# cvg/pixel-perfect-sfm

Hardware: AMD Instinct MI355X
Metric: featuremetric residuals+Jacobians evaluated/sec (1M obs) (higher is better)
Workload: dtype f32 horizontal / f64 vertical+normalisation on f16 patches; 1 GPU; BASELINE.json configs[2]: synthetic 200 cams / 200000 points / 1000000 obs featuremetric BA residual+Jacobian evaluation, 128-ch fp16 16x16 patches, SIMPLE_RADIAL, fused six-scalar Jacobian reduction; n_obs=1000000, channels=128, patch=16, obs_per_gpu=1000000, partition=none

## Files before the change

### pixel-perfect-sfm_amd/csrc/pxr_ba_gram.hip

```cpp
#include <hip/hip_runtime.h>

#include <algorithm>

#include "pxr_ba_solve.h"
#include "pxr_device.h"
#include "pxr_gram.h"
#include "pxr_internal.h"

namespace pxr {

constexpr int GC_STRIDE = IG_GDOUBLES + 16;

struct GramArgs {
  pxr_ba_view v;
  const void* arena; const int32_t* corners; const double* scales;
  int H, W, l2_normalize;
  double* G;
  int2* cell;
  int* dirty;
  const double* r2;
  double* rec;
};

template <typename ST, int C>
__global__ __launch_bounds__(64) void k_gram_build(const GramArgs a) {
  __shared__ double refbuf[3][C];
  const int lane = threadIdx.x;
  const ST* arena = reinterpret_cast<const ST*>(a.arena);
  const size_t patch_elems = (size_t)a.H * a.W * C;
  const int64_t n = a.v.n_obs;
  for (int64_t base = (int64_t)blockIdx.x * 64; base < n; base += (int64_t)gridDim.x * 64) {
    const int64_t o = min(base + lane, n - 1);
    unsigned long long todo = __ballot(base + lane < n && a.dirty[o] != 0);
    if (todo == 0ull) continue;
    const int64_t pidx = a.v.d_obs_patch[o];
    const int pt = a.v.d_obs_point[o];
    const int2 cl = a.cell[o];
    const int pi_lo = (int)(pidx & 0xffffffffll), pi_hi = (int)(pidx >> 32);
    double2 rr0 = make_double2(0.0, 0.0), rr1 = rr0, rr2 = rr0;
    auto take = [&](GramTexels<ST, C>& tx, double2& rr) -> int {
      if (todo == 0ull) return -1;
      const int j = __ffsll((long long)todo) - 1;
      todo &= todo - 1ull;
      const int row = __builtin_amdgcn_readlane(cl.x, j), col = __builtin_amdgcn_readlane(cl.y, j);
      const int64_t pi = ((int64_t)__builtin_amdgcn_readlane(pi_hi, j) << 32) | (unsigned)__builtin_amdgcn_readlane(pi_lo, j);
      const int p = __builtin_amdgcn_readlane(pt, j);
#ifdef PXR_GRAM_PROBE_NO_LOAD
      tx.load(arena, a.H, a.W, 5, 5);
#else
      tx.load(arena + (size_t)pi * patch_elems, a.H, a.W, row, col);
#endif
      if (2 * lane < C) rr = *reinterpret_cast<const double2*>(a.v.d_refs + (size_t)p * C + 2 * lane);
      return j;
    };
    auto build = [&](const GramTexels<ST, C>& tx, const double2& rr, int slot, int j) {
      if (2 * lane < C) *reinterpret_cast<double2*>(&refbuf[slot][2 * lane]) = rr;
      __syncthreads();
      double* g = a.G + (size_t)(base + j) * GC_STRIDE;
      gram_contract<ST, C>(tx, refbuf[slot], g, g + IG_GDOUBLES);
    };
    GramTexels<ST, C> t0, t1, t2;
    int s0 = take(t0, rr0), s1 = take(t1, rr1), s2 = take(t2, rr2);
    while (true) {
      if (s0 < 0) break;
      build(t0, rr0, 0, s0); s0 = take(t0, rr0);
      if (s1 < 0) break;
      build(t1, rr1, 1, s1); s1 = take(t1, rr1);
      if (s2 < 0) break;
      build(t2, rr2, 2, s2); s2 = take(t2, rr2);
    }
  }
}

template <bool FIRST>
__device__ __forceinline__ void gram_eval_eight(const GramArgs& a, double* S, int64_t i, int nq, int lane) {
  const int q = lane >> 3, sub = lane & 7, ri = sub >> 1, ci = 2 * (sub & 1);
  constexpr int NT = (8 * GC_STRIDE / 2 + 63) / 64, PER = GC_STRIDE / 2;
  static_assert(NT * 64 == 8 * PER, "the last request stays inside the buffer");
  const int n2 = nq * PER;
#pragma unroll
  for (int j = 0; j < NT; ++j) {
    const int e = min(lane + 64 * j, n2 - 1);
    const double2* src;
    if (FIRST) {
      src = reinterpret_cast<const double2*>(a.G + (size_t)__shfl((int)i, 0) * GC_STRIDE) + e;
    } else {
      const int64_t oi = __shfl((int)i, 8 * (e / PER));
      src = reinterpret_cast<const double2*>(a.G + (size_t)oi * GC_STRIDE) + e % PER;
    }
    __builtin_amdgcn_global_load_lds((const __attribute__((address_space(1))) void*)src,
                                     (__attribute__((address_space(3))) void*)(S + 2 * 64 * j), 16, 0, 0);
  }
  const int img = a.v.d_obs_image[i];
  const int pt = a.v.d_obs_point[i];
  const int64_t pidx = a.v.d_obs_patch[i];
  int2 cached = make_int2(0, 0);
  if (FIRST) cached = a.cell[i];
  const int cam = a.v.d_image_camera[img];
  double qv[4], t[3], X[3], k[PXR_KPAD];
#pragma unroll
  for (int j = 0; j < 4; ++j) qv[j] = a.v.d_qvec[4 * (size_t)img + j];
#pragma unroll
  for (int j = 0; j < 3; ++j) { t[j] = a.v.d_tvec[3 * (size_t)img + j]; X[j] = a.v.d_xyz[3 * (size_t)pt + j]; }
#pragma unroll
  for (int j = 0; j < PXR_KPAD; ++j) k[j] = a.v.d_cam_params[(size_t)cam * PXR_KPAD + j];
  const double sx = a.scales[2 * pidx], sy = a.scales[2 * pidx + 1];
  const double cx = (double)a.corners[2 * pidx], cy = (double)a.corners[2 * pidx + 1];
  const double r2 = a.r2[pt];
  double x, y;
  world_to_pixel(a.v.d_cam_model[cam], k, qv, t, X, x, y);
  const double u = x * sx - 0.5 - cx, v = y * sy - 0.5 - cy;
  const double rf = floor(v), cf = floor(u);
  const int row = texel_index(rf, a.H), col = texel_index(cf, a.W);
  const bool miss = FIRST && (cached.x != row || cached.y != col);
  if (FIRST && q < nq && sub == 0) {
    a.dirty[i] = miss ? 1 : 0;
    if (miss) a.cell[i] = make_int2(row, col);
  }
  double wu[4], dwu[4], wv[4], dwv[4];
  catmull_rom_weights(u - cf, wu, dwu);
  catmull_rom_weights(v - rf, wv, dwv);
  __builtin_amdgcn_s_waitcnt(0x0f70);
  __syncthreads();
  if (q >= nq || miss) return;
  const double* Gq = S + (size_t)q * GC_STRIDE;
  double ya[3], yb[3];
  gram_rows_times_weights(Gq, sub, wu, dwu, wv, dwv, ya, yb);
  const double2 d2 = *reinterpret_cast<const double2*>(Gq + IG_GDOUBLES + 2 * sub);
  const double wvo = pick4(wv, ri), dwvo = pick4(dwv, ri);
  const double wua = ci == 0 ? wu[0] : wu[2], wub = ci == 0 ? wu[1] : wu[3];
  const double dwua = ci == 0 ? dwu[0] : dwu[2], dwub = ci == 0 ? dwu[1] : dwu[3];
  const double oma = wvo * wua, omb = wvo * wub, omca = wvo * dwua, omcb = wvo * dwub, omra = dwvo * wua, omrb = dwvo * wub;
  const double Sgg = row8_sum(fma(oma, ya[0], omb * yb[0])), Sgc = row8_sum(fma(oma, ya[1], omb * yb[1]));
  const double Sgr = row8_sum(fma(oma, ya[2], omb * yb[2]));
  const double Scc = row8_sum(fma(omca, ya[1], omcb * yb[1])), Scr = row8_sum(fma(omca, ya[2], omcb * yb[2]));
  const double Srr = row8_sum(fma(omra, ya[2], omrb * yb[2]));
  const double Sfd = row8_sum(fma(oma, d2.x, omb * d2.y)), Scd = row8_sum(fma(omca, d2.x, omcb * d2.y));
  const double Srd = row8_sum(fma(omra, d2.x, omrb * d2.y));
  if (sub != 0) return;
  double s, gcc, gcr, grr, bc, br;
  if (a.l2_normalize) {
    const double ninv = 1.0 / sqrt(Sgg), n2inv = ninv * ninv;
    const double pc = Sgc * n2inv, pr = Sgr * n2inv;
    s = 1.0 - 2.0 * Sfd * ninv + r2;
    gcc = (Scc - Sgc * pc) * n2inv; gcr = (Scr - Sgc * pr) * n2inv; grr = (Srr - Sgr * pr) * n2inv;
    bc = -(Scd - Sfd * pc) * ninv; br = -(Srd - Sfd * pr) * ninv;
  } else {
    s = Sgg - 2.0 * Sfd + r2;
    gcc = Scc; gcr = Scr; grr = Srr; bc = Sgc - Scd; br = Sgr - Srd;
  }
  if (s < 0.0) s = 0.0;
  double2* out = reinterpret_cast<double2*>(a.rec + (size_t)i * PXR_OBS_REC);
  out[0] = make_double2(s, gcc * sx * sx);
  out[1] = make_double2(gcr * sx * sy, grr * sy * sy);
  out[2] = make_double2(bc * sx, br * sy);
  out[3] = make_double2(x, y);
}

__global__ __launch_bounds__(64) void k_gram_eval(const GramArgs a) {
  __shared__ __align__(16) double S[8 * GC_STRIDE];
  const int lane = threadIdx.x;
  const int64_t o0 = (int64_t)blockIdx.x * 8;
  const int nq = (int)min<int64_t>(8, a.v.n_obs - o0);
  if (nq <= 0) return;
  gram_eval_eight<true>(a, S, o0 + min(lane >> 3, nq - 1), nq, lane);
}

__global__ __launch_bounds__(64) void k_gram_eval_dirty(const GramArgs a) {
  __shared__ __align__(16) double S[8 * GC_STRIDE];
  const int lane = threadIdx.x;
  const int64_t base = (int64_t)blockIdx.x * 64, n = a.v.n_obs;
  unsigned long long todo = __ballot(base + lane < n && a.dirty[min(base + lane, n - 1)] != 0);
#pragma clang loop unroll(disable)
  while (todo != 0ull) {
    const int nq = min(8, __popcll(todo));
    unsigned long long m = todo;
    for (int t = min(lane >> 3, nq - 1); t > 0; --t) m &= m - 1ull;
    const int64_t i = base + __ffsll((long long)m) - 1;
    gram_eval_eight<false>(a, S, i, nq, lane);
    for (int t = 0; t < nq; ++t) todo &= todo - 1ull;
    __syncthreads();
  }
}

__global__ __launch_bounds__(256) void k_gram_count_dirty(int64_t n, const int* __restrict__ dirty, int* __restrict__ count) {
  const int64_t i = (int64_t)blockIdx.x * blockDim.x + threadIdx.x;
  const unsigned long long m = __ballot(i < n && dirty[min(i, n - 1)] != 0);
  if ((threadIdx.x & 63) == 0 && m != 0ull) atomicAdd(count, __popcll(m));
}

__global__ __launch_bounds__(256) void k_gram_r2(int64_t n_pts, int C, const double* __restrict__ refs, double* __restrict__ r2) {
  const int64_t t = (int64_t)blockIdx.x * blockDim.x + threadIdx.x;
  const int64_t p = t >> 4;
  const int sub = (int)(t & 15);
  double acc = 0.0;
  if (p < n_pts)
    for (int ch = sub; ch < C; ch += 16) { const double d = refs[(size_t)p * C + ch]; acc = fma(d, d, acc); }
  acc = row16_sum(acc);
  if (p < n_pts && sub == 0) r2[p] = acc;
}

__global__ __launch_bounds__(256) void k_gram_invalidate(int64_t n, int2* __restrict__ cell) {
  const int64_t i = (int64_t)blockIdx.x * blockDim.x + threadIdx.x;
  if (i < n) cell[i] = make_int2(-1000000, -1000000);
}

bool gram_eval_supported(const pxr_arena* arena, const pxr_ba_view* view) {
  return view->d_refs != nullptr && (arena->C == 128 || arena->C == 64) && (arena->dtype == PXR_F16 || arena->dtype == PXR_F32) &&
         arena->up == 1.0 && view->n_obs > 0 && view->n_obs < (int64_t)1 << 31;
}

static size_t align256(size_t b) { return (b + 255) & ~(size_t)255; }

static void gram_layout(void* base, int64_t n, int64_t np, GramCache* out, size_t* total) {
  const size_t bG = align256(sizeof(double) * (size_t)n * GC_STRIDE), bcell = align256(sizeof(int2) * (size_t)n),
               blist = align256(sizeof(int) * (size_t)n), bcount = 256, br2 = align256(sizeof(double) * (size_t)np);
  char* p = static_cast<char*>(base);
  out->G = reinterpret_cast<double*>(p); p += bG;
  out->cell = p; p += bcell;
  out->list = reinterpret_cast<int*>(p); p += blist;
  out->count = reinterpret_cast<int*>(p); p += bcount;
  out->r2 = reinterpret_cast<double*>(p);
  out->n_obs = n;
  *total = bG + bcell + blist + bcount + br2;
}

int gram_eval_prepare(pxr_ctx* ctx, pxr_arena* arena, const pxr_ba_view* view, GramCache* out) {
  const int64_t n = view->n_obs, np = view->n_points;
  size_t need = 0;
  gram_layout(nullptr, n, np, out, &need);
  if (ctx->gram_bytes < need) {
    if (ctx->d_gram) PXR_HIP(hipFree(ctx->d_gram));
    ctx->d_gram = nullptr; ctx->gram_bytes = 0;
    if (getenv("PXR_GRAM_FAIL_ALLOC") != nullptr || hipMalloc(&ctx->d_gram, need) != hipSuccess) { (void)hipGetLastError(); return set_error(PXR_ENOMEM, "Gram-matrix cache: %zu bytes", need); }
    ctx->gram_bytes = need;
  }
  gram_layout(ctx->d_gram, n, np, out, &need);
  hipStream_t st = ctx->stream;
  hipLaunchKernelGGL(k_gram_invalidate, dim3((unsigned)((n + 255) / 256)), dim3(256), 0, st, n, static_cast<int2*>(out->cell));
  hipLaunchKernelGGL(k_gram_r2, dim3((unsigned)((np * 16 + 255) / 256)), dim3(256), 0, st, np, arena->C, view->d_refs, out->r2);
  return hip_check(hipGetLastError(), "Gram-matrix cache set-up");
}

int gram_build_flagged(pxr_ctx* ctx, pxr_arena* arena, const pxr_ba_view* v, const GramCache& gc) {
  GramArgs a;
  a.v = *v;
  a.arena = arena->d_data; a.corners = arena->d_corners; a.scales = arena->d_scales;
  a.H = arena->H; a.W = arena->W; a.l2_normalize = 0;
  a.G = gc.G; a.cell = static_cast<int2*>(gc.cell); a.dirty = gc.list; a.r2 = gc.r2; a.rec = nullptr;
  const int64_t n = v->n_obs;
  const unsigned build_grid = (unsigned)std::min<int64_t>((n + 63) / 64, (int64_t)ctx->num_cus * 16);
#define GRAM_BUILD(ST, CC) hipLaunchKernelGGL((k_gram_build<ST, CC>), dim3(build_grid), dim3(64), 0, ctx->stream, a)
  if (arena->dtype == PXR_F16) { if (arena->C == 128) GRAM_BUILD(_Float16, 128); else GRAM_BUILD(_Float16, 64); }
  else { if (arena->C == 128) GRAM_BUILD(float, 128); else GRAM_BUILD(float, 64); }
#undef GRAM_BUILD
  return hip_check(hipGetLastError(), "Gram-matrix build");
}

int gram_evaluate(pxr_ctx* ctx, pxr_arena* arena, const pxr_ba_view* v, const pxr_interp_cfg* cfg, const GramCache& gc, double* rec) {
  GramArgs a;
  a.v = *v;
  a.arena = arena->d_data; a.corners = arena->d_corners; a.scales = arena->d_scales;
  a.H = arena->H; a.W = arena->W; a.l2_normalize = cfg->l2_normalize;
  a.G = gc.G; a.cell = static_cast<int2*>(gc.cell); a.dirty = gc.list; a.r2 = gc.r2; a.rec = rec;
  hipStream_t st = ctx->stream;
  const int64_t n = v->n_obs;
  hipLaunchKernelGGL(k_gram_eval, dim3((unsigned)((n + 7) / 8)), dim3(64), 0, st, a);
  const unsigned build_grid = (unsigned)std::min<int64_t>((n + 63) / 64, (int64_t)ctx->num_cus * 16);
#define GRAM_BUILD(ST, CC) hipLaunchKernelGGL((k_gram_build<ST, CC>), dim3(build_grid), dim3(64), 0, st, a)
  if (arena->dtype == PXR_F16) { if (arena->C == 128) GRAM_BUILD(_Float16, 128); else GRAM_BUILD(_Float16, 64); }
  else { if (arena->C == 128) GRAM_BUILD(float, 128); else GRAM_BUILD(float, 64); }
#undef GRAM_BUILD
  hipLaunchKernelGGL(k_gram_eval_dirty, dim3((unsigned)((n + 63) / 64)), dim3(64), 0, st, a);
  return hip_check(hipGetLastError(), "Gram-matrix evaluation");
}

}

extern "C" int pxr_ba_eval_gram(pxr_ctx* ctx, pxr_arena* arena, const pxr_ba_view* view, const pxr_interp_cfg* cfg, int reset,
                                double* d_rec, int32_t* h_rebuilt) {
  using namespace pxr;
  PXR_REQUIRE(ctx && arena && view && cfg && d_rec, "pxr_ba_eval_gram: NULL argument");
  PXR_REQUIRE(gram_eval_supported(arena, view), "pxr_ba_eval_gram: needs feature patches of 128 / 64 channels in fp16 / fp32 storage and reference descriptors");
  PXR_HIP(hipSetDevice(ctx->device));
  GramCache gc;
  size_t need = 0;
  gram_layout(ctx->d_gram, view->n_obs, view->n_points, &gc, &need);
  if (reset || ctx->gram_bytes < need) {
    if (int rc = gram_eval_prepare(ctx, arena, view, &gc)) return rc;
  }
  if (int rc = gram_evaluate(ctx, arena, view, cfg, gc, d_rec)) return rc;
  if (h_rebuilt) {
    PXR_HIP(hipMemsetAsync(gc.count, 0, sizeof(int), ctx->stream));
    hipLaunchKernelGGL(k_gram_count_dirty, dim3((unsigned)((view->n_obs + 255) / 256)), dim3(256), 0, ctx->stream, view->n_obs, gc.list, gc.count);
    PXR_HIP(hipMemcpyAsync(h_rebuilt, gc.count, sizeof(int32_t), hipMemcpyDeviceToHost, ctx->stream));
    PXR_HIP(hipStreamSynchronize(ctx->stream));
  }
  return PXR_OK;
}
```

### pixel-perfect-sfm_amd/csrc/pxr_ba_inner.hip

```cpp
#include <hip/hip_runtime.h>

#include <cstdlib>
#include <type_traits>
#include <vector>
#include <algorithm>

#include "pxr_device.h"
#include "pxr_gram.h"
#include "pxr_interp.h"
#include "pxr_internal.h"

namespace pxr {

struct InnerArgs {
  pxr_ba_view v;
  const void* arena; const int32_t* corners; const double* scales; int H, W;
  int l2_normalize, check_bounds;
  double up;
  pxr_loss loss;
  const int64_t* pt_ptr; const int64_t* pt_obs; const int* pt_var;
  double* xyz_out;
  double* cost_before;
  double* cost_pt;
  double* gram_G;
// ... 897 lines not shown
      inner_owner_update(S, rs[0], Hc, gc, first, true, active, a.cost_before, a.cost_pt ? a.cost_pt + p : nullptr);
    }
    first = false;
    GQ_MARK(5);
#ifdef PXR_INNER_PROFILE
    ++gq_rounds;
#endif
    if (__builtin_amdgcn_readfirstlane((int)active) == 0) break;
  }
#ifdef PXR_INNER_PROFILE
  if ((blockIdx.x == 1000 || blockIdx.x == 150000) && lane == 0)
    printf("[inner gram profile, wavefront %d, 100 MHz ticks x 10 ns] rounds %d builds %d  staging %lld  projection %lld  gram builds %lld  evaluation %lld  reduce %lld  owner LM %lld\n",
           (int)blockIdx.x, gq_rounds, gq_builds, gq_acc[0], gq_acc[1], gq_acc[2], gq_acc[3], gq_acc[4], gq_acc[5]);
#endif
  if (variable && lane == 0) { a.xyz_out[3 * p] = S.X[0]; a.xyz_out[3 * p + 1] = S.X[1]; a.xyz_out[3 * p + 2] = S.X[2]; }
}

struct GramWave { int npts, pad; int p[IP_MAXPTS]; int st[IP_MAXPTS + 1]; int pad2; };
static_assert(sizeof(GramWave) == 48, "table layout");
constexpr int GW_SLOTS = 16;
__host__ __device__ inline size_t gram_wave_bytes() { return sizeof(GramWave) + sizeof(GramSlot) * GW_SLOTS; }
#ifndef PXR_GW_GPAD
#define PXR_GW_GPAD 4
#endif
struct GramWaveLds {
  double G[GW_SLOTS][IG_GDOUBLES + PXR_GW_GPAD];
  double D[GW_SLOTS][16];
  double obs[GW_SLOTS][IG_OBS];
  double res[GW_SLOTS][10];
  double refbuf[128];
  InnerOwner own[IP_MAXPTS];
};

__global__ __launch_bounds__(256) void k_gram_wave_table(int64_t n_waves, const GramWave* __restrict__ waves, const int64_t* __restrict__ pt_ptr,
                                                         const int64_t* __restrict__ pt_obs, const int32_t* __restrict__ obs_image,
                                                         const int64_t* __restrict__ obs_patch, const int32_t* __restrict__ image_camera,
                                                         char* __restrict__ table) {
  const int64_t t = (int64_t)blockIdx.x * blockDim.x + threadIdx.x;
  const int64_t e = t / (GW_SLOTS + 1);
  const int q = (int)(t % (GW_SLOTS + 1)) - 1;
  if (e >= n_waves) return;
  const GramWave w = waves[e];
  char* ent = table + (size_t)e * gram_wave_bytes();
  if (q < 0) { *reinterpret_cast<GramWave*>(ent) = w; return; }
  const int L = w.st[w.npts];
  const int qc = min(q, L - 1);
  int j = 0;
  while (j + 1 < w.npts && qc >= w.st[j + 1]) ++j;
  const int64_t i = pt_obs[pt_ptr[w.p[j]] + (qc - w.st[j])];
  const int img = obs_image[i];
  reinterpret_cast<GramSlot*>(ent + sizeof(GramWave))[q] = GramSlot{img, image_camera[img], obs_patch[i], i};
}

__global__ __launch_bounds__(256) void k_gram_flag_slots(const InnerArgs a, const char* __restrict__ table, int64_t n_waves, int* __restrict__ dirty) {
  const int64_t t = (int64_t)blockIdx.x * blockDim.x + threadIdx.x;
  const int64_t e = t / GW_SLOTS;
  const int q = (int)(t % GW_SLOTS);
  if (e >= n_waves) return;
  const char* ent = table + (size_t)e * gram_wave_bytes();
  const GramWave* gw = reinterpret_cast<const GramWave*>(ent);
  const int npts = gw->npts, L = gw->st[npts];
  if (q >= L) return;
  int j = 0;
  while (j + 1 < npts && q >= gw->st[j + 1]) ++j;
  const int64_t p = gw->p[j];
  const GramSlot sl = reinterpret_cast<const GramSlot*>(ent + sizeof(GramWave))[q];
  double qv[4], tv[3], X[3], k[PXR_KPAD];
#pragma unroll
  for (int m = 0; m < 4; ++m) qv[m] = a.v.d_qvec[4 * (size_t)sl.img + m];
#pragma unroll
  for (int m = 0; m < 3; ++m) { tv[m] = a.v.d_tvec[3 * (size_t)sl.img + m]; X[m] = a.v.d_xyz[3 * (size_t)p + m]; }
#pragma unroll
  for (int m = 0; m < PXR_KPAD; ++m) k[m] = a.v.d_cam_params[(size_t)sl.cam * PXR_KPAD + m];
  double R[9];
  quat_to_rotation(qv, R);
  const double p0 = fma(R[0], X[0], fma(R[1], X[1], fma(R[2], X[2], tv[0])));
  const double p1 = fma(R[3], X[0], fma(R[4], X[1], fma(R[5], X[2], tv[1])));
  const double p2 = fma(R[6], X[0], fma(R[7], X[1], fma(R[8], X[2], tv[2])));
  const double iz = inner_rcp(p2), un = p0 * iz, vn = p1 * iz;
  double x, y, Juv[2][2];
  camera_model_jac<false, false>(a.v.d_cam_model[sl.cam], k, un, vn, x, y, Juv, nullptr);
  const double u = x * a.scales[2 * sl.patch] - 0.5 - (double)a.corners[2 * sl.patch];
  const double v = y * a.scales[2 * sl.patch + 1] - 0.5 - (double)a.corners[2 * sl.patch + 1];
  const int row = texel_index(floor(v), a.H), col = texel_index(floor(u), a.W);
  const int2 c = a.gram_cell[sl.obs];
  const bool miss = c.x != row || c.y != col;
  dirty[sl.obs] = miss ? 1 : 0;
  if (miss) a.gram_cell[sl.obs] = make_int2(row, col);
}

template <typename ST, int C>
__global__ __launch_bounds__(64) __attribute__((amdgpu_waves_per_eu(2, 2))) void k_inner_gram_packed(const InnerArgs a, const char* __restrict__ table) {
  static_assert(C == 128 || C == 64, "feature patches");
  __shared__ __align__(16) GramWaveLds lds;
  const int lane = threadIdx.x, sidx = lane >> 2, sub = lane & 3;
  const char* const ent = table + (size_t)blockIdx.x * gram_wave_bytes();
  const GramWave* const gw = reinterpret_cast<const GramWave*>(ent);
  const GramSlot* const slots = reinterpret_cast<const GramSlot*>(ent + sizeof(GramWave));
  const GramSlot sl = slots[sidx];
  const int npts = gw->npts, L = gw->st[npts];
  const int st1 = gw->st[1 < npts ? 1 : npts], st2 = gw->st[2 < npts ? 2 : npts], st3 = gw->st[3 < npts ? 3 : npts];
  const bool owner = lane < npts;
  const int64_t myp = gw->p[owner ? lane : 0];
  const int my_b = owner ? gw->st[lane] : 0, my_e = owner ? gw->st[lane + 1] : 0;
  const bool variable = owner && a.pt_var[myp] != 0;
  bool active = variable, first = true;
  const ST* arena = reinterpret_cast<const ST*>(a.arena);
  const size_t patch_elems = (size_t)a.H * a.W * C;
  const bool l2 = a.l2_normalize != 0;
  const bool warm = a.gram_G != nullptr && a.gram_warm != 0;
  const int q = sidx;
  const bool valid = q < L;
  const int jq = ((valid ? q : L - 1) >= st1) + ((valid ? q : L - 1) >= st2) + ((valid ? q : L - 1) >= st3);

  const int hi = lane < 24 ? lane : 23;
  double2 va0, va1, va2, va3, va4, va5, va6, va7, vb0, vb1, vb2, vb3, vb4, vb5, vb6, vb7;
#define GW_FETCH(Q0, J, VA, VB)                                                                                       \
  {                                                                                                                   \
    const int64_t oi = __shfl((int)sl.obs, 4 * min(Q0 + J, L - 1));              \
    const double2* g = reinterpret_cast<const double2*>(a.gram_G + (size_t)oi * (IG_GDOUBLES + 16));                   \
    VA = g[lane]; VB = g[64 + hi];                                                                                    \
  }
#define GW_PUT(Q0, J, VA, VB)                                                                                         \
  if (Q0 + J < L) {                                                                                                   \
    double2* Gd = reinterpret_cast<double2*>(lds.G[Q0 + J]);                                                          \
    Gd[lane] = VA;                                                                                                    \
    if (lane < 16) Gd[64 + lane] = VB;                                                                                \
    else if (lane < 24) reinterpret_cast<double2*>(lds.D[Q0 + J])[lane - 16] = VB;                                    \
  }
#define GW_FETCH8(Q0) GW_FETCH(Q0, 0, va0, vb0) GW_FETCH(Q0, 1, va1, vb1) GW_FETCH(Q0, 2, va2, vb2) GW_FETCH(Q0, 3, va3, vb3) \
                      GW_FETCH(Q0, 4, va4, vb4) GW_FETCH(Q0, 5, va5, vb5) GW_FETCH(Q0, 6, va6, vb6) GW_FETCH(Q0, 7, va7, vb7)
#define GW_PUT8(Q0) GW_PUT(Q0, 0, va0, vb0) GW_PUT(Q0, 1, va1, vb1) GW_PUT(Q0, 2, va2, vb2) GW_PUT(Q0, 3, va3, vb3) \
                    GW_PUT(Q0, 4, va4, vb4) GW_PUT(Q0, 5, va5, vb5) GW_PUT(Q0, 6, va6, vb6) GW_PUT(Q0, 7, va7, vb7)
  if (warm) { GW_FETCH8(0) }
  if (valid) {
    double* ob = lds.obs[q];
    const int img = sl.img, cam = sl.cam;
    const int64_t pi = sl.patch;
    if (sub == 0) {
// ... 240 lines not shown
  a.arena = arena->d_data; a.corners = arena->d_corners; a.scales = arena->d_scales;
  a.H = arena->H; a.W = arena->W; a.up = arena->up; a.l2_normalize = cfg->l2_normalize; a.check_bounds = cfg->check_bounds; a.loss = *loss;
  a.pt_ptr = d_pt_ptr; a.pt_obs = d_pt_obs; a.pt_var = d_pt_var;
  a.xyz_out = const_cast<double*>(view->d_xyz); a.cost_before = d_cost_before; a.cost_pt = d_cost_per_point;
  a.gram_G = gram ? gram->G : nullptr; a.gram_cell = gram ? static_cast<int2*>(gram->cell) : nullptr; a.gram_warm = gram_warm ? 1 : 0;
  const int ppb = arena->C >= 64 ? 1 : 8;
  const int threads = 64;
  const unsigned blocks = (unsigned)((view->n_points + ppb - 1) / ppb);
  if (blocks == 0) return PXR_OK;
#define INNER_LAUNCH(KERNEL, ST, CC)                                                                          \
  do {                                                                                                        \
    if (cfg->use_float_simd) hipLaunchKernelGGL((KERNEL<ST, CC, true>), dim3(blocks), dim3(threads), 0, ctx->stream, a);  \
    else hipLaunchKernelGGL((KERNEL<ST, CC, false>), dim3(blocks), dim3(threads), 0, ctx->stream, a);             \
  } while (0)
#define INNER_PACKED(ST, CC, NBLK, PPW, LIST)                                                                             \
  do {                                                                                                                    \
    if (cfg->use_float_simd) hipLaunchKernelGGL((k_inner_packed<ST, CC, true, 4>), dim3(NBLK), dim3(64), 0, ctx->stream, a, PPW, LIST);  \
    else hipLaunchKernelGGL((k_inner_packed<ST, CC, false, 4>), dim3(NBLK), dim3(64), 0, ctx->stream, a, PPW, LIST);         \
  } while (0)
#define INNER_BY_STORAGE(MACRO, ...)                                                    \
  do {                                                                                  \
    if (arena->dtype == PXR_F16 && arena->C == 128) MACRO(_Float16, 128, __VA_ARGS__);  \
    else if (arena->dtype == PXR_F16) MACRO(_Float16, 64, __VA_ARGS__);                 \
    else if (arena->C == 128) MACRO(float, 128, __VA_ARGS__);                           \
    else MACRO(float, 64, __VA_ARGS__);                                                 \
  } while (0)
#define INNER_GRAM(ST, CC, NBLK, MAXO)                                                                                    \
  hipLaunchKernelGGL((k_inner_gram<ST, CC>), dim3(NBLK), dim3(64), sizeof(double) * gram_lds_doubles(MAXO, CC), ctx->stream, a, \
                     static_cast<const char*>(lists->d_slots), MAXO)
#define INNER_GRAM_PACKED(ST, CC, NBLK) \
  hipLaunchKernelGGL((k_inner_gram_packed<ST, CC>), dim3(NBLK), dim3(64), 0, ctx->stream, a, static_cast<const char*>(lists->d_waves))
  if (arena->C <= 4) {
    if (arena->dtype == PXR_F16 && arena->C == 3) INNER_LAUNCH(k_inner_points, _Float16, 3);
    else if (arena->dtype == PXR_F16) INNER_LAUNCH(k_inner_points, _Float16, 1);
    else if (arena->dtype == PXR_F32 && arena->C == 3) INNER_LAUNCH(k_inner_points, float, 3);
    else if (arena->dtype == PXR_F32) INNER_LAUNCH(k_inner_points, float, 1);
    else if (arena->C == 3) INNER_LAUNCH(k_inner_points, double, 3);
    else INNER_LAUNCH(k_inner_points, double, 1);
  } else if (getenv("PXR_INNER_OLD")) {
    if (arena->dtype == PXR_F16 && arena->C == 128) INNER_LAUNCH(k_inner_points, _Float16, 128);
    else if (arena->dtype == PXR_F16) INNER_LAUNCH(k_inner_points, _Float16, 64);
    else if (arena->dtype == PXR_F32 && arena->C == 128) INNER_LAUNCH(k_inner_points, float, 128);
    else if (arena->dtype == PXR_F32) INNER_LAUNCH(k_inner_points, float, 64);
    else if (arena->C == 128) INNER_LAUNCH(k_inner_points, double, 128);
    else INNER_LAUNCH(k_inner_points, double, 64);
  } else if (arena->dtype != PXR_F64) {
    if (lists == nullptr || getenv("PXR_INNER_PACKED")) {
      const int64_t per16 = view->n_obs > 0 ? (16 * view->n_points) / view->n_obs : 1;
      const int ppw = (int)(per16 < 1 ? 1 : (per16 > IP_MAXPTS ? IP_MAXPTS : per16));
      const unsigned pblocks = (unsigned)((view->n_points + ppw - 1) / ppw);
      const int* no_list = nullptr;
      INNER_BY_STORAGE(INNER_PACKED, pblocks, ppw, no_list);
    } else {
      if (lists->n_waves > 0) {
        if (gram && !getenv("PXR_INNER_NO_PREBUILD")) {
          PXR_HIP(hipMemsetAsync(gram->list, 0, sizeof(int) * (size_t)view->n_obs, ctx->stream));
          const int64_t n_thr = lists->n_waves * GW_SLOTS;
          hipLaunchKernelGGL(k_gram_flag_slots, dim3((unsigned)((n_thr + 255) / 256)), dim3(256), 0, ctx->stream, a, static_cast<const char*>(lists->d_waves),
                             lists->n_waves, gram->list);
          if (int rc = gram_build_flagged(ctx, arena, view, *gram)) return rc;
          a.gram_warm = 1;
        }
        INNER_BY_STORAGE(INNER_GRAM_PACKED, (unsigned)lists->n_waves);
      }
      else if (lists->n_short > 0 && lists->d_slots) INNER_BY_STORAGE(INNER_GRAM, (unsigned)lists->n_short, lists->maxo_short);
      if (lists->n_long > 0) INNER_BY_STORAGE(INNER_PACKED, (unsigned)lists->n_long, 1, lists->d_long);
    }
  } else if (arena->dtype == PXR_F64 && arena->C == 128) INNER_LAUNCH(k_inner_points, double, 128);
  else INNER_LAUNCH(k_inner_points, double, 64);
#undef INNER_LAUNCH
#undef INNER_PACKED
#undef INNER_GRAM
#undef INNER_GRAM_PACKED
#undef INNER_BY_STORAGE
  return hip_check(hipGetLastError(), "k_inner_points launch");
}

size_t inner_wave_stage_bytes(int64_t n_pts) { return sizeof(GramWave) * (size_t)(n_pts + 1); }
int make_inner_lists(pxr_ctx* ctx, const int64_t* pt_ptr, int64_t n, void* h_wave_stage, size_t wave_stage_bytes, const pxr_ba_view* view,
                     const int64_t* d_pt_ptr, const int64_t* d_pt_obs, InnerLists* out) {
  hipStream_t st = ctx->stream;
  const bool one_point_kernel = getenv("PXR_INNER_GRAM1") != nullptr;
  std::vector<GramPoint> shorts;
  std::vector<GramWave> waves_pageable;
  GramWave* wv = wave_stage_bytes >= inner_wave_stage_bytes(n) ? static_cast<GramWave*>(h_wave_stage) : nullptr;
  int64_t n_wv = 0;
  std::vector<int> longs;
  int maxo = 1;
  const int max_pts = getenv("PXR_INNER_GRAM_PPW") ? std::max(1, std::min(IP_MAXPTS, atoi(getenv("PXR_INNER_GRAM_PPW")))) : IP_MAXPTS;
  if (one_point_kernel) shorts.reserve((size_t)n); else if (!wv) waves_pageable.reserve((size_t)n / 2 + 1);
  int64_t n_short = 0;
  GramWave cur{};
  auto flush = [&]() {
    if (cur.npts > 0) { if (wv) wv[n_wv] = cur; else waves_pageable.push_back(cur); ++n_wv; }
    cur = GramWave{};
  };
  for (int64_t p = 0; p < n; ++p) {
    const int64_t len = pt_ptr[p + 1] - pt_ptr[p];
    if (len <= 0) continue;
    if (len <= IG_MAXO) {
      ++n_short; maxo = std::max(maxo, (int)len);
      if (one_point_kernel) { shorts.push_back(GramPoint{(int)p, (int)len, pt_ptr[p]}); continue; }
      if (cur.npts == max_pts || cur.st[cur.npts] + (int)len > GW_SLOTS) flush();
      cur.p[cur.npts] = (int)p;
      cur.st[cur.npts + 1] = cur.st[cur.npts] + (int)len;
      ++cur.npts;
    } else longs.push_back((int)p);
  }
  flush();
  const GramWave* const waves = wv ? wv : waves_pageable.data();
  out->n_waves = n_wv; out->d_waves = nullptr; out->d_wave_heads = nullptr;
  out->n_short = n_short; out->n_long = (int64_t)longs.size(); out->maxo_short = maxo;
// ... 40 lines not shown
```

### pixel-perfect-sfm_amd/csrc/pxr_gram.h

```cpp
#pragma once
#include <hip/hip_runtime.h>

#include <type_traits>

#include "pxr_device.h"
#include "pxr_interp.h"

namespace pxr {

typedef double gd4 __attribute__((ext_vector_type(4)));

__device__ __forceinline__ void catmull_rom_weights(double x, double (&w)[4], double (&dw)[4]) {
  const double x2 = x * x, x3 = x2 * x;
  w[0] = -0.5 * x + x2 - 0.5 * x3; w[1] = 1.0 - 2.5 * x2 + 1.5 * x3; w[2] = 0.5 * x + 2.0 * x2 - 1.5 * x3; w[3] = -0.5 * x2 + 0.5 * x3;
  dw[0] = -0.5 + 2.0 * x - 1.5 * x2; dw[1] = -5.0 * x + 4.5 * x2; dw[2] = 0.5 + 4.0 * x - 4.5 * x2; dw[3] = -x + 1.5 * x2;
}
__device__ __forceinline__ double pick4(const double (&w)[4], int i) { return i == 0 ? w[0] : (i == 1 ? w[1] : (i == 2 ? w[2] : w[3])); }

template <typename ST, int C>
struct GramTexels {
  static constexpr int CPL = C / 4;
  static constexpr int VPL = sizeof(ST) == 2 ? 8 : 4;
  typename std::conditional<sizeof(ST) == 2, uint4, float4>::type raw[CPL / VPL];
  static __device__ __forceinline__ int channel(int g, int e) { return (e / VPL) * (4 * VPL) + g * VPL + e % VPL; }
// ... 31 lines not shown
  double dp = 0.0;
#pragma unroll
  for (int e = 0; e < CPL; e += 2) {
    const double x0 = tx.value(e), x1 = tx.value(e + 1);
#ifdef PXR_GRAM_PROBE_NO_MFMA
    acc0[0] += x0; acc1[0] += x1;
#else
    acc0 = __builtin_amdgcn_mfma_f64_16x16x4f64(x0, x0, acc0, 0, 0, 0);
    acc1 = __builtin_amdgcn_mfma_f64_16x16x4f64(x1, x1, acc1, 0, 0, 0);
#endif
    dp = fma(x0, ref[GramTexels<ST, C>::channel(g, e)], dp);
    dp = fma(x1, ref[GramTexels<ST, C>::channel(g, e + 1)], dp);
  }
  dp += __shfl_xor(dp, 16);
  dp += __shfl_xor(dp, 32);
  if (g == 0) Dq[i] = dp;
  const gd4 acc = acc0 + acc1;
  const int cb = i >> 2, ic = i & 3;
#pragma unroll
  for (int r = 0; r < 4; ++r)
    if (cb >= r) Gq[gram_block(r, cb) * 16 + g * 4 + ic] = acc[r];
}

__device__ __forceinline__ void gram_rows_times_weights(const double* Gq, int sub, const double (&wu)[4], const double (&dwu)[4],
                                                        const double (&wv)[4], const double (&dwv)[4], double (&ya)[3], double (&yb)[3]) {
  const int R = sub >> 1, ir = 2 * (sub & 1);
  ya[0] = ya[1] = ya[2] = yb[0] = yb[1] = yb[2] = 0.0;
#pragma unroll
  for (int cbk = 0; cbk < 4; ++cbk) {
    double ea[4], eb[4];
    if (cbk >= R) {
      const double* blk = Gq + gram_block(R, cbk) * 16 + ir * 4;
      const double2 a01 = *reinterpret_cast<const double2*>(blk), a23 = *reinterpret_cast<const double2*>(blk + 2);
      const double2 b01 = *reinterpret_cast<const double2*>(blk + 4), b23 = *reinterpret_cast<const double2*>(blk + 6);
      ea[0] = a01.x; ea[1] = a01.y; ea[2] = a23.x; ea[3] = a23.y; eb[0] = b01.x; eb[1] = b01.y; eb[2] = b23.x; eb[3] = b23.y;
    } else {
      const double* blk = Gq + gram_block(cbk, R) * 16 + ir;
#pragma unroll
      for (int cc = 0; cc < 4; ++cc) {
        const double2 t = *reinterpret_cast<const double2*>(blk + 4 * cc);
        ea[cc] = t.x; eb[cc] = t.y;
      }
    }
    const double za = fma(ea[3], wu[3], fma(ea[2], wu[2], fma(ea[1], wu[1], ea[0] * wu[0])));
    const double zb = fma(eb[3], wu[3], fma(eb[2], wu[2], fma(eb[1], wu[1], eb[0] * wu[0])));
    const double zca = fma(ea[3], dwu[3], fma(ea[2], dwu[2], fma(ea[1], dwu[1], ea[0] * dwu[0])));
    const double zcb = fma(eb[3], dwu[3], fma(eb[2], dwu[2], fma(eb[1], dwu[1], eb[0] * dwu[0])));
    ya[0] = fma(wv[cbk], za, ya[0]); yb[0] = fma(wv[cbk], zb, yb[0]);
    ya[1] = fma(wv[cbk], zca, ya[1]); yb[1] = fma(wv[cbk], zcb, yb[1]);
    ya[2] = fma(dwv[cbk], za, ya[2]); yb[2] = fma(dwv[cbk], zb, yb[2]);
  }
}

}
```

### pixel-perfect-sfm_amd/csrc/pxr_internal.h

```cpp
#pragma once
#include <hip/hip_runtime.h>

#include <cstdarg>
#include <cstdio>
#include <string>

#include "pixsfm_hip.h"

struct pxr_ctx {
  int device = 0;
  hipStream_t stream = nullptr;
  hipEvent_t ev_start = nullptr, ev_stop = nullptr;
  hipEvent_t ev_sync = nullptr;
  void* h_readback = nullptr;
  void* h_setup = nullptr;
  size_t h_setup_bytes = 0;
  double* d_scratch = nullptr;
  size_t scratch_bytes = 0;
  int num_cus = 256;
  void* d_workspace = nullptr;
  size_t workspace_bytes = 0;
  void* d_workspace_mat = nullptr;
  size_t workspace_mat_bytes = 0;
  void* comm = nullptr;
  int rank = 0, nranks = 1;
  bool force_collective = false;
  int64_t collective_calls = 0;
  int64_t collective_bytes = 0;
  pxr_iteration_callback iter_cb = nullptr;
  void* iter_user = nullptr;
  void* h_stage[2] = {nullptr, nullptr};
  hipEvent_t ev_stage[2] = {nullptr, nullptr};
  size_t stage_bytes = 0;
  bool deterministic = true;
  bool gram_cache = true;
  void* d_gram = nullptr;
  size_t gram_bytes = 0;
  void* d_solve_arena = nullptr;
  size_t solve_arena_bytes = 0;
};

struct pxr_arena {
  pxr_ctx* ctx = nullptr;
  int dtype = PXR_F16, C = 0, H = 0, W = 0;
  int64_t n = 0;
  void* d_data = nullptr;
  bool owns_data = false;
  int32_t* d_corners = nullptr;
  double* d_scales = nullptr;
  double up = 1.0;
  size_t elem_size() const { return dtype == PXR_F16 ? 2 : (dtype == PXR_F32 ? 4 : 8); }
  size_t patch_bytes() const { return (size_t)H * W * C * elem_size(); }
};

namespace pxr {
int set_error(int code, const char* fmt, ...);
inline int hip_check(hipError_t e, const char* what) {
  if (e == hipSuccess) return PXR_OK;
  return set_error(PXR_EHIP, "%s: %s", what, hipGetErrorString(e));
}
void* setup_staging(pxr_ctx* ctx, size_t bytes);
int comm_allreduce_sum(pxr_ctx* ctx, double* d_buf, int64_t count, bool even_single_rank = false);
int comm_allreduce_sum_i64(pxr_ctx* ctx, long long* d_buf, int64_t count);
int ba_eval_with_cost(pxr_ctx* ctx, pxr_arena* arena, const pxr_ba_view* view, const pxr_interp_cfg* cfg,
                      int with_jacobian, double* d_rec, double* d_r, double* d_gx, double* d_gy,
                      const pxr_loss* loss, double* d_cost_sum);
int geom_eval(pxr_ctx* ctx, const pxr_ba_view* view, const double* d_obs_xy, double* d_rec, double* d_res);
int launch_inner_geom(pxr_ctx* ctx, const pxr_ba_view* view, const double* d_obs_xy, const pxr_loss* loss, const int64_t* d_pt_ptr,
                      const int64_t* d_pt_obs, const int* d_pt_var, double* d_cost_before, double* d_cost_per_point,
                      bool extended_models);
struct InnerLists {
  void* d_short = nullptr; int64_t n_short = 0; int maxo_short = 1;
  int* d_long = nullptr; int64_t n_long = 0;
  void* d_slots = nullptr;
  void* d_waves = nullptr; int64_t n_waves = 0;
  void* d_wave_heads = nullptr;
  bool own_short = true, own_long = true, own_slots = true, own_heads = true;
};
void* solve_scratch(size_t bytes, bool* owned);
struct GramCache {
  double* G = nullptr;
  void* cell = nullptr;
  int* list = nullptr;
  int* count = nullptr;
  double* r2 = nullptr;
  int64_t n_obs = 0;
};
bool gram_eval_supported(const pxr_arena* arena, const pxr_ba_view* view);
int gram_eval_prepare(pxr_ctx* ctx, pxr_arena* arena, const pxr_ba_view* view, GramCache* out);
int gram_evaluate(pxr_ctx* ctx, pxr_arena* arena, const pxr_ba_view* v, const pxr_interp_cfg* cfg, const GramCache& gc, double* rec);
// ... 14 lines not shown
```

Before: 1.436 billion residual_blocks/s.

## Fuse Gram build with evaluation and skip cached-cell checks on cold cache

Adds a fused kernel that builds the per-observation Gram blocks in shared memory and evaluates the residual and Jacobian record straight from them, then writes the blocks back to the cache. A 'cold' flag set at cache preparation lets the first evaluation skip the separate eval pass and mark every observation dirty without reading stale cells. The aim is to remove a separate eval launch and the re-read of G from global memory after the build. The fused kernel is on by default through an environment variable and raises register and LDS pressure, with waves-per-EU forced to 3 or 4.

```diff
diff --git a/pixel-perfect-sfm_amd/csrc/pxr_ba_gram.hip b/pixel-perfect-sfm_amd/csrc/pxr_ba_gram.hip
--- a/pixel-perfect-sfm_amd/csrc/pxr_ba_gram.hip
+++ b/pixel-perfect-sfm_amd/csrc/pxr_ba_gram.hip
@@ -1,6 +1,7 @@
 #include <hip/hip_runtime.h>
 
 #include <algorithm>
+#include <cstdlib>
 
 #include "pxr_ba_solve.h"
 #include "pxr_device.h"
@@ -8,19 +9,6 @@
 #include "pxr_internal.h"
 
 namespace pxr {
-
-constexpr int GC_STRIDE = IG_GDOUBLES + 16;
-
-struct GramArgs {
-  pxr_ba_view v;
-  const void* arena; const int32_t* corners; const double* scales;
-  int H, W, l2_normalize;
-  double* G;
-  int2* cell;
-  int* dirty;
-  const double* r2;
-  double* rec;
-};
 
 template <typename ST, int C>
 __global__ __launch_bounds__(64) void k_gram_build(const GramArgs a) {
@@ -72,9 +60,8 @@
   }
 }
 
-template <bool FIRST>
-__device__ __forceinline__ void gram_eval_eight(const GramArgs& a, double* S, int64_t i, int nq, int lane) {
-  const int q = lane >> 3, sub = lane & 7, ri = sub >> 1, ci = 2 * (sub & 1);
+template <bool CONTIGUOUS>
+__device__ __forceinline__ void gram_request_eight(const GramArgs& a, double* S, int64_t i, int nq, int lane) {
   constexpr int NT = (8 * GC_STRIDE / 2 + 63) / 64, PER = GC_STRIDE / 2;
   static_assert(NT * 64 == 8 * PER, "the last request stays inside the buffer");
   const int n2 = nq * PER;
@@ -82,7 +69,7 @@
   for (int j = 0; j < NT; ++j) {
     const int e = min(lane + 64 * j, n2 - 1);
     const double2* src;
-    if (FIRST) {
+    if (CONTIGUOUS) {
       src = reinterpret_cast<const double2*>(a.G + (size_t)__shfl((int)i, 0) * GC_STRIDE) + e;
     } else {
       const int64_t oi = __shfl((int)i, 8 * (e / PER));
@@ -91,70 +78,25 @@
     __builtin_amdgcn_global_load_lds((const __attribute__((address_space(1))) void*)src,
                                      (__attribute__((address_space(3))) void*)(S + 2 * 64 * j), 16, 0, 0);
   }
-  const int img = a.v.d_obs_image[i];
-  const int pt = a.v.d_obs_point[i];
-  const int64_t pidx = a.v.d_obs_patch[i];
+}
+
+template <bool FIRST>
+__device__ __forceinline__ void gram_eval_eight(const GramArgs& a, double* S, int64_t i, int nq, int lane) {
+  const int q = lane >> 3, sub = lane & 7;
+  gram_request_eight<FIRST>(a, S, i, nq, lane);
   int2 cached = make_int2(0, 0);
   if (FIRST) cached = a.cell[i];
-  const int cam = a.v.d_image_camera[img];
-  double qv[4], t[3], X[3], k[PXR_KPAD];
-#pragma unroll
-  for (int j = 0; j < 4; ++j) qv[j] = a.v.d_qvec[4 * (size_t)img + j];
-#pragma unroll
-  for (int j = 0; j < 3; ++j) { t[j] = a.v.d_tvec[3 * (size_t)img + j]; X[j] = a.v.d_xyz[3 * (size_t)pt + j]; }
-#pragma unroll
-  for (int j = 0; j < PXR_KPAD; ++j) k[j] = a.v.d_cam_params[(size_t)cam * PXR_KPAD + j];
-  const double sx = a.scales[2 * pidx], sy = a.scales[2 * pidx + 1];
-  const double cx = (double)a.corners[2 * pidx], cy = (double)a.corners[2 * pidx + 1];
-  const double r2 = a.r2[pt];
-  double x, y;
-  world_to_pixel(a.v.d_cam_model[cam], k, qv, t, X, x, y);
-  const double u = x * sx - 0.5 - cx, v = y * sy - 0.5 - cy;
-  const double rf = floor(v), cf = floor(u);
-  const int row = texel_index(rf, a.H), col = texel_index(cf, a.W);
-  const bool miss = FIRST && (cached.x != row || cached.y != col);
+  GramProj p;
+  gram_project(a, i, p);
+  const bool miss = FIRST && (cached.x != p.row || cached.y != p.col);
   if (FIRST && q < nq && sub == 0) {
     a.dirty[i] = miss ? 1 : 0;
-    if (miss) a.cell[i] = make_int2(row, col);
-  }
-  double wu[4], dwu[4], wv[4], dwv[4];
-  catmull_rom_weights(u - cf, wu, dwu);
-  catmull_rom_weights(v - rf, wv, dwv);
+    if (miss) a.cell[i] = make_int2(p.row, p.col);
+  }
   __builtin_amdgcn_s_waitcnt(0x0f70);
   __syncthreads();
   if (q >= nq || miss) return;
-  const double* Gq = S + (size_t)q * GC_STRIDE;
-  double ya[3], yb[3];
-  gram_rows_times_weights(Gq, sub, wu, dwu, wv, dwv, ya, yb);
-  const double2 d2 = *reinterpret_cast<const double2*>(Gq + IG_GDOUBLES + 2 * sub);
-  const double wvo = pick4(wv, ri), dwvo = pick4(dwv, ri);
-  const double wua = ci == 0 ? wu[0] : wu[2], wub = ci == 0 ? wu[1] : wu[3];
-  const double dwua = ci == 0 ? dwu[0] : dwu[2], dwub = ci == 0 ? dwu[1] : dwu[3];
-  const double oma = wvo * wua, omb = wvo * wub, omca = wvo * dwua, omcb = wvo * dwub, omra = dwvo * wua, omrb = dwvo * wub;
-  const double Sgg = row8_sum(fma(oma, ya[0], omb * yb[0])), Sgc = row8_sum(fma(oma, ya[1], omb * yb[1]));
-  const double Sgr = row8_sum(fma(oma, ya[2], omb * yb[2]));
-  const double Scc = row8_sum(fma(omca, ya[1], omcb * yb[1])), Scr = row8_sum(fma(omca, ya[2], omcb * yb[2]));
-  const double Srr = row8_sum(fma(omra, ya[2], omrb * yb[2]));
-  const double Sfd = row8_sum(fma(oma, d2.x, omb * d2.y)), Scd = row8_sum(fma(omca, d2.x, omcb * d2.y));
-  const double Srd = row8_sum(fma(omra, d2.x, omrb * d2.y));
-  if (sub != 0) return;
-  double s, gcc, gcr, grr, bc, br;
-  if (a.l2_normalize) {
-    const double ninv = 1.0 / sqrt(Sgg), n2inv = ninv * ninv;
-    const double pc = Sgc * n2inv, pr = Sgr * n2inv;
-    s = 1.0 - 2.0 * Sfd * ninv + r2;
-    gcc = (Scc - Sgc * pc) * n2inv; gcr = (Scr - Sgc * pr) * n2inv; grr = (Srr - Sgr * pr) * n2inv;
-    bc = -(Scd - Sfd * pc) * ninv; br = -(Srd - Sfd * pr) * ninv;
-  } else {
-    s = Sgg - 2.0 * Sfd + r2;
-    gcc = Scc; gcr = Scr; grr = Srr; bc = Sgc - Scd; br = Sgr - Srd;
-  }
-  if (s < 0.0) s = 0.0;
-  double2* out = reinterpret_cast<double2*>(a.rec + (size_t)i * PXR_OBS_REC);
-  out[0] = make_double2(s, gcc * sx * sx);
-  out[1] = make_double2(gcr * sx * sy, grr * sy * sy);
-  out[2] = make_double2(bc * sx, br * sy);
-  out[3] = make_double2(x, y);
+  gram_record(a, S + (size_t)q * GC_STRIDE, p, i, sub);
 }
 
 __global__ __launch_bounds__(64) void k_gram_eval(const GramArgs a) {
@@ -239,6 +181,7 @@
   hipStream_t st = ctx->stream;
   hipLaunchKernelGGL(k_gram_invalidate, dim3((unsigned)((n + 255) / 256)), dim3(256), 0, st, n, static_cast<int2*>(out->cell));
   hipLaunchKernelGGL(k_gram_r2, dim3((unsigned)((np * 16 + 255) / 256)), dim3(256), 0, st, np, arena->C, view->d_refs, out->r2);
+  ctx->gram_cold = true;
   return hip_check(hipGetLastError(), "Gram-matrix cache set-up");
 }
 
@@ -248,6 +191,7 @@
   a.arena = arena->d_data; a.corners = arena->d_corners; a.scales = arena->d_scales;
   a.H = arena->H; a.W = arena->W; a.l2_normalize = 0;
   a.G = gc.G; a.cell = static_cast<int2*>(gc.cell); a.dirty = gc.list; a.r2 = gc.r2; a.rec = nullptr;
+  ctx->gram_cold = false;
   const int64_t n = v->n_obs;
   const unsigned build_grid = (unsigned)std::min<int64_t>((n + 63) / 64, (int64_t)ctx->num_cus * 16);
 #define GRAM_BUILD(ST, CC) hipLaunchKernelGGL((k_gram_build<ST, CC>), dim3(build_grid), dim3(64), 0, ctx->stream, a)
@@ -256,6 +200,9 @@
 #undef GRAM_BUILD
   return hip_check(hipGetLastError(), "Gram-matrix build");
 }
+
+int gram_launch_build_eval(pxr_ctx* ctx, const pxr_arena* arena, const GramArgs& a, bool all, bool four);
+static bool gram_fused() { const char* e = getenv("PXR_GRAM_FUSED"); return e == nullptr || atoi(e) != 0; }
 
 int gram_evaluate(pxr_ctx* ctx, pxr_arena* arena, const pxr_ba_view* v, const pxr_interp_cfg* cfg, const GramCache& gc, double* rec) {
   GramArgs a;
@@ -265,8 +212,15 @@
   a.G = gc.G; a.cell = static_cast<int2*>(gc.cell); a.dirty = gc.list; a.r2 = gc.r2; a.rec = rec;
   hipStream_t st = ctx->stream;
   const int64_t n = v->n_obs;
-  hipLaunchKernelGGL(k_gram_eval, dim3((unsigned)((n + 7) / 8)), dim3(64), 0, st, a);
+  const bool fused = gram_fused();
+  const bool cold = fused && ctx->gram_cold;
+  ctx->gram_cold = false;
+  if (!cold) hipLaunchKernelGGL(k_gram_eval, dim3((unsigned)((n + 7) / 8)), dim3(64), 0, st, a);
   const unsigned build_grid = (unsigned)std::min<int64_t>((n + 63) / 64, (int64_t)ctx->num_cus * 16);
+  if (fused) {
+    const char* ge = getenv("PXR_GRAM_FUSED_GROUP");
+    return gram_launch_build_eval(ctx, arena, a, cold, ge != nullptr && atoi(ge) == 4);
+  }
 #define GRAM_BUILD(ST, CC) hipLaunchKernelGGL((k_gram_build<ST, CC>), dim3(build_grid), dim3(64), 0, st, a)
   if (arena->dtype == PXR_F16) { if (arena->C == 128) GRAM_BUILD(_Float16, 128); else GRAM_BUILD(_Float16, 64); }
   else { if (arena->C == 128) GRAM_BUILD(float, 128); else GRAM_BUILD(float, 64); }
diff --git a/pixel-perfect-sfm_amd/csrc/pxr_ba_gram_fused.hip b/pixel-perfect-sfm_amd/csrc/pxr_ba_gram_fused.hip
--- /dev/null
+++ b/pixel-perfect-sfm_amd/csrc/pxr_ba_gram_fused.hip
@@ -0,0 +1,117 @@
+#include <hip/hip_runtime.h>
+
+#include <algorithm>
+
+#include "pxr_ba_solve.h"
+#include "pxr_device.h"
+#include "pxr_gram.h"
+#include "pxr_internal.h"
+
+namespace pxr {
+
+template <typename ST, int C, bool ALL, int GRP>
+__global__ __launch_bounds__(64) __attribute__((amdgpu_waves_per_eu(GRP <= 4 ? 4 : 3, GRP <= 4 ? 4 : 3))) void k_gram_build_eval(const GramArgs a) {
+  static_assert(GRP >= 1 && GRP <= 8, "8 lanes per observation");
+  __shared__ __align__(16) double S[GRP * GC_STRIDE];
+  __shared__ double refbuf[3][C];
+  const int lane = threadIdx.x;
+  const ST* arena = reinterpret_cast<const ST*>(a.arena);
+  const size_t patch_elems = (size_t)a.H * a.W * C;
+  const int64_t n = a.v.n_obs;
+  constexpr int PER = GC_STRIDE / 2, NT = (GRP * PER + 63) / 64;
+  for (int64_t base = (int64_t)blockIdx.x * 64; base < n; base += (int64_t)gridDim.x * 64) {
+    const int64_t o = min(base + lane, n - 1);
+    const bool valid = base + lane < n;
+    unsigned long long left;
+    int2 cl;
+    if (ALL) {
+      GramProj p;
+      gram_project(a, o, p);
+      cl = make_int2(p.row, p.col);
+      if (valid) { a.dirty[o] = 1; a.cell[o] = cl; }
+      left = __ballot(valid);
+    } else {
+      left = __ballot(valid && a.dirty[o] != 0);
+      if (left == 0ull) continue;
+      cl = a.cell[o];
+    }
+    const int64_t pidx = a.v.d_obs_patch[o];
+    const int pt = a.v.d_obs_point[o];
+    const int pi_lo = (int)(pidx & 0xffffffffll), pi_hi = (int)(pidx >> 32);
+#pragma clang loop unroll(disable)
+    while (left != 0ull) {
+      const int nq = min(GRP, __popcll(left));
+      unsigned long long todo = left;
+      int nreq = 0, nbuilt = 0;
+      double2 rr0 = make_double2(0.0, 0.0), rr1 = rr0, rr2 = rr0;
+      auto take = [&](GramTexels<ST, C>& tx, double2& rr) -> bool {
+        if (nreq == nq) return false;
+        ++nreq;
+        const int j = __ffsll((long long)todo) - 1;
+        todo &= todo - 1ull;
+        const int row = __builtin_amdgcn_readlane(cl.x, j), col = __builtin_amdgcn_readlane(cl.y, j);
+        const int64_t pi = ((int64_t)__builtin_amdgcn_readlane(pi_hi, j) << 32) | (unsigned)__builtin_amdgcn_readlane(pi_lo, j);
+        const int p = __builtin_amdgcn_readlane(pt, j);
+        tx.load(arena + (size_t)pi * patch_elems, a.H, a.W, row, col);
+        if (2 * lane < C) rr = *reinterpret_cast<const double2*>(a.v.d_refs + (size_t)p * C + 2 * lane);
+        return true;
+      };
+      auto build = [&](const GramTexels<ST, C>& tx, const double2& rr, int slot) {
+        if (2 * lane < C) *reinterpret_cast<double2*>(&refbuf[slot][2 * lane]) = rr;
+        __syncthreads();
+        double* g = S + (size_t)nbuilt * GC_STRIDE;
+        gram_contract<ST, C>(tx, refbuf[slot], g, g + IG_GDOUBLES);
+        ++nbuilt;
+      };
+      {
+        GramTexels<ST, C> t0, t1, t2;
+        bool s0 = take(t0, rr0), s1 = take(t1, rr1), s2 = take(t2, rr2);
+        while (true) {
+          if (!s0) break;
+          build(t0, rr0, 0); s0 = take(t0, rr0);
+          if (!s1) break;
+          build(t1, rr1, 1); s1 = take(t1, rr1);
+          if (!s2) break;
+          build(t2, rr2, 2); s2 = take(t2, rr2);
+        }
+      }
+      __syncthreads();
+      unsigned long long m = left;
+      for (int t = min(lane >> 3, nq - 1); t > 0; --t) m &= m - 1ull;
+      const int off = __ffsll((long long)m) - 1;
+      if ((lane >> 3) < nq) {
+        GramProj p;
+        gram_project(a, base + off, p);
+        gram_record(a, S + (size_t)(lane >> 3) * GC_STRIDE, p, base + off, lane & 7);
+      }
+#pragma unroll
+      for (int j = 0; j < NT; ++j) {
+        const int e = lane + 64 * j, ec = min(e, nq * PER - 1);
+        const int oe = __shfl(off, 8 * (ec / PER));
+        if (e < nq * PER)
+          reinterpret_cast<double2*>(a.G + (size_t)(base + oe) * GC_STRIDE)[ec % PER] = reinterpret_cast<const double2*>(S)[ec];
+      }
+      for (int t = 0; t < nq; ++t) left &= left - 1ull;
+      __syncthreads();
+    }
+  }
+}
+
+int gram_launch_build_eval(pxr_ctx* ctx, const pxr_arena* arena, const GramArgs& a, bool all, bool four) {
+  const int64_t n = a.v.n_obs;
+  const unsigned grid = (unsigned)std::min<int64_t>((n + 63) / 64, (int64_t)ctx->num_cus * 16);
+  hipStream_t st = ctx->stream;
+#define GRAM_FUSED(ST, CC)                                                                                          \
+  do {                                                                                                              \
+    if (all) { if (four) hipLaunchKernelGGL((k_gram_build_eval<ST, CC, true, 4>), dim3(grid), dim3(64), 0, st, a);   \
+               else hipLaunchKernelGGL((k_gram_build_eval<ST, CC, true, 8>), dim3(grid), dim3(64), 0, st, a); }      \
+    else { if (four) hipLaunchKernelGGL((k_gram_build_eval<ST, CC, false, 4>), dim3(grid), dim3(64), 0, st, a);      \
+           else hipLaunchKernelGGL((k_gram_build_eval<ST, CC, false, 8>), dim3(grid), dim3(64), 0, st, a); }         \
+  } while (0)
+  if (arena->dtype == PXR_F16) { if (arena->C == 128) GRAM_FUSED(_Float16, 128); else GRAM_FUSED(_Float16, 64); }
+  else { if (arena->C == 128) GRAM_FUSED(float, 128); else GRAM_FUSED(float, 64); }
+#undef GRAM_FUSED
+  return hip_check(hipGetLastError(), "Gram-matrix build + evaluation");
+}
+
+}
diff --git a/pixel-perfect-sfm_amd/csrc/pxr_ba_inner.hip b/pixel-perfect-sfm_amd/csrc/pxr_ba_inner.hip
--- a/pixel-perfect-sfm_amd/csrc/pxr_ba_inner.hip
+++ b/pixel-perfect-sfm_amd/csrc/pxr_ba_inner.hip
@@ -973,6 +973,7 @@
   reinterpret_cast<GramSlot*>(ent + sizeof(GramWave))[q] = GramSlot{img, image_camera[img], obs_patch[i], i};
 }
 
+template <bool COLD>
 __global__ __launch_bounds__(256) void k_gram_flag_slots(const InnerArgs a, const char* __restrict__ table, int64_t n_waves, int* __restrict__ dirty) {
   const int64_t t = (int64_t)blockIdx.x * blockDim.x + threadIdx.x;
   const int64_t e = t / GW_SLOTS;
@@ -1004,8 +1005,8 @@
   const double u = x * a.scales[2 * sl.patch] - 0.5 - (double)a.corners[2 * sl.patch];
   const double v = y * a.scales[2 * sl.patch + 1] - 0.5 - (double)a.corners[2 * sl.patch + 1];
   const int row = texel_index(floor(v), a.H), col = texel_index(floor(u), a.W);
-  const int2 c = a.gram_cell[sl.obs];
-  const bool miss = c.x != row || c.y != col;
+  bool miss = true;
+  if (!COLD) { const int2 c = a.gram_cell[sl.obs]; miss = c.x != row || c.y != col; }
   dirty[sl.obs] = miss ? 1 : 0;
   if (miss) a.gram_cell[sl.obs] = make_int2(row, col);
 }
@@ -1352,12 +1353,18 @@
       const int* no_list = nullptr;
       INNER_BY_STORAGE(INNER_PACKED, pblocks, ppw, no_list);
     } else {
+      const bool cold = ctx->gram_cold;
+      if (gram && (lists->n_waves > 0 || (lists->n_short > 0 && lists->d_slots))) ctx->gram_cold = false;
       if (lists->n_waves > 0) {
         if (gram && !getenv("PXR_INNER_NO_PREBUILD")) {
           PXR_HIP(hipMemsetAsync(gram->list, 0, sizeof(int) * (size_t)view->n_obs, ctx->stream));
           const int64_t n_thr = lists->n_waves * GW_SLOTS;
-          hipLaunchKernelGGL(k_gram_flag_slots, dim3((unsigned)((n_thr + 255) / 256)), dim3(256), 0, ctx->stream, a, static_cast<const char*>(lists->d_waves),
-                             lists->n_waves, gram->list);
+          if (cold)
+            hipLaunchKernelGGL(k_gram_flag_slots<true>, dim3((unsigned)((n_thr + 255) / 256)), dim3(256), 0, ctx->stream, a,
+                               static_cast<const char*>(lists->d_waves), lists->n_waves, gram->list);
+          else
+            hipLaunchKernelGGL(k_gram_flag_slots<false>, dim3((unsigned)((n_thr + 255) / 256)), dim3(256), 0, ctx->stream, a,
+                               static_cast<const char*>(lists->d_waves), lists->n_waves, gram->list);
           if (int rc = gram_build_flagged(ctx, arena, view, *gram)) return rc;
           a.gram_warm = 1;
         }
diff --git a/pixel-perfect-sfm_amd/csrc/pxr_gram.h b/pixel-perfect-sfm_amd/csrc/pxr_gram.h
--- a/pixel-perfect-sfm_amd/csrc/pxr_gram.h
+++ b/pixel-perfect-sfm_amd/csrc/pxr_gram.h
@@ -107,4 +107,82 @@
   }
 }
 
+constexpr int GC_STRIDE = IG_GDOUBLES + 16;
+
+struct GramArgs {
+  pxr_ba_view v;
+  const void* arena; const int32_t* corners; const double* scales;
+  int H, W, l2_normalize;
+  double* G;
+  int2* cell;
+  int* dirty;
+  const double* r2;
+  double* rec;
+};
+
+struct GramProj {
+  double x, y, sx, sy, r2;
+  int row, col;
+  double wu[4], dwu[4], wv[4], dwv[4];
+};
+__device__ __forceinline__ void gram_project(const GramArgs& a, int64_t i, GramProj& p) {
+  const int img = a.v.d_obs_image[i];
+  const int pt = a.v.d_obs_point[i];
+  const int64_t pidx = a.v.d_obs_patch[i];
+  const int cam = a.v.d_image_camera[img];
+  double qv[4], t[3], X[3], k[PXR_KPAD];
+#pragma unroll
+  for (int j = 0; j < 4; ++j) qv[j] = a.v.d_qvec[4 * (size_t)img + j];
+#pragma unroll
+  for (int j = 0; j < 3; ++j) { t[j] = a.v.d_tvec[3 * (size_t)img + j]; X[j] = a.v.d_xyz[3 * (size_t)pt + j]; }
+#pragma unroll
+  for (int j = 0; j < PXR_KPAD; ++j) k[j] = a.v.d_cam_params[(size_t)cam * PXR_KPAD + j];
+  p.sx = a.scales[2 * pidx]; p.sy = a.scales[2 * pidx + 1];
+  const double cx = (double)a.corners[2 * pidx], cy = (double)a.corners[2 * pidx + 1];
+  p.r2 = a.r2[pt];
+  world_to_pixel(a.v.d_cam_model[cam], k, qv, t, X, p.x, p.y);
+  const double u = p.x * p.sx - 0.5 - cx, v = p.y * p.sy - 0.5 - cy;
+  const double rf = floor(v), cf = floor(u);
+  p.row = texel_index(rf, a.H); p.col = texel_index(cf, a.W);
+  catmull_rom_weights(u - cf, p.wu, p.dwu);
+  catmull_rom_weights(v - rf, p.wv, p.dwv);
 }
+
+__device__ __forceinline__ void gram_record(const GramArgs& a, const double* Gq, const GramProj& p, int64_t i, int sub) {
+  const int ri = sub >> 1, ci = 2 * (sub & 1);
+  const double (&wu)[4] = p.wu, (&dwu)[4] = p.dwu, (&wv)[4] = p.wv, (&dwv)[4] = p.dwv;
+  const double sx = p.sx, sy = p.sy;
+  double ya[3], yb[3];
+  gram_rows_times_weights(Gq, sub, wu, dwu, wv, dwv, ya, yb);
+  const double2 d2 = *reinterpret_cast<const double2*>(Gq + IG_GDOUBLES + 2 * sub);
+  const double wvo = pick4(wv, ri), dwvo = pick4(dwv, ri);
+  const double wua = ci == 0 ? wu[0] : wu[2], wub = ci == 0 ? wu[1] : wu[3];
+  const double dwua = ci == 0 ? dwu[0] : dwu[2], dwub = ci == 0 ? dwu[1] : dwu[3];
+  const double oma = wvo * wua, omb = wvo * wub, omca = wvo * dwua, omcb = wvo * dwub, omra = dwvo * wua, omrb = dwvo * wub;
+  const double Sgg = row8_sum(fma(oma, ya[0], omb * yb[0])), Sgc = row8_sum(fma(oma, ya[1], omb * yb[1]));
+  const double Sgr = row8_sum(fma(oma, ya[2], omb * yb[2]));
+  const double Scc = row8_sum(fma(omca, ya[1], omcb * yb[1])), Scr = row8_sum(fma(omca, ya[2], omcb * yb[2]));
+  const double Srr = row8_sum(fma(omra, ya[2], omrb * yb[2]));
+  const double Sfd = row8_sum(fma(oma, d2.x, omb * d2.y)), Scd = row8_sum(fma(omca, d2.x, omcb * d2.y));
+  const double Srd = row8_sum(fma(omra, d2.x, omrb * d2.y));
+  if (sub != 0) return;
+  double s, gcc, gcr, grr, bc, br;
+  if (a.l2_normalize) {
+    const double ninv = 1.0 / sqrt(Sgg), n2inv = ninv * ninv;
+    const double pc = Sgc * n2inv, pr = Sgr * n2inv;
+    s = 1.0 - 2.0 * Sfd * ninv + p.r2;
+    gcc = (Scc - Sgc * pc) * n2inv; gcr = (Scr - Sgc * pr) * n2inv; grr = (Srr - Sgr * pr) * n2inv;
+    bc = -(Scd - Sfd * pc) * ninv; br = -(Srd - Sfd * pr) * ninv;
+  } else {
+    s = Sgg - 2.0 * Sfd + p.r2;
+    gcc = Scc; gcr = Scr; grr = Srr; bc = Sgc - Scd; br = Sgr - Srd;
+  }
+  if (s < 0.0) s = 0.0;
+  double2* out = reinterpret_cast<double2*>(a.rec + (size_t)i * PXR_OBS_REC);
+  out[0] = make_double2(s, gcc * sx * sx);
+  out[1] = make_double2(gcr * sx * sy, grr * sy * sy);
+  out[2] = make_double2(bc * sx, br * sy);
+  out[3] = make_double2(p.x, p.y);
+}
+
+}
diff --git a/pixel-perfect-sfm_amd/csrc/pxr_internal.h b/pixel-perfect-sfm_amd/csrc/pxr_internal.h
--- a/pixel-perfect-sfm_amd/csrc/pxr_internal.h
+++ b/pixel-perfect-sfm_amd/csrc/pxr_internal.h
@@ -36,6 +36,7 @@
   bool gram_cache = true;
   void* d_gram = nullptr;
   size_t gram_bytes = 0;
+  bool gram_cold = false;
   void* d_solve_arena = nullptr;
   size_t solve_arena_bytes = 0;
 };
```

Result: no change. 1.429 billion residual_blocks/s (-0.5%).
